# iancze/PSOAP

Hardware: AMD Instinct MI355X
Metric: GP lnprob evals/sec (SB2, N=6000) (higher is better)
Workload: dtype f64; 1 GPU; SB2 chunk 20 epochs x 300 px (N=6000), 32 walkers per step per GPU, one chunk per GPU (BASELINE.json configs[2]; configs[3] at 8 GPUs); timed step = H2D of next proposals || eval, D2H of 32 lnprobs, gather; N=6000, components=2, walkers=32, chunks_per_gpu=1, mode=dag, stream_groups=2, parallelism=chunk-sharded x1, RCCL all_gather of walker lnprobs

## Files before the change

include/psoap_gp.h:

```cpp
#ifndef PSOAP_GP_H
#define PSOAP_GP_H

#include <stdint.h>

#ifdef __cplusplus
extern "C" {
#endif

typedef struct psoap_chunk psoap_chunk;

int psoap_version(void);
const char *psoap_last_error(void);
int psoap_device_count(int *count);

enum {
    PSOAP_SHARE_PROCS = 0,
    PSOAP_SHARE_DAG_LAUNCHES = 1,
    PSOAP_SHARE_TAINTED = 2,
    PSOAP_SHARE_RETRIES = 3,
    PSOAP_SHARE_STAGED_FALLBACKS = 4,
    PSOAP_SHARE_STAGED_POLICY = 5,
    PSOAP_SHARE_MOVED_TASKS = 6,
    PSOAP_SHARE_MOVED_XCD = 7,
    PSOAP_SHARE_LOCK_ACQUISITIONS = 8,
// ... 176 lines not shown
int psoap_stream_plan(int P, int lanes, int workers, int scheme, void *out, long long max_tasks, long long *n_tasks,
                      long long *n_slots, long long *n_ctrs, int *scheme_out);
int psoap_stream_tasklog(psoap_chunk *h, int cap, unsigned long long *out, long long max_words);
int psoap_stream_tasks(psoap_chunk *h, void *out, long long max_tasks, long long *n_tasks);

int psoap_chunk_dag_tasks(psoap_chunk *h, void *out, long long max_tasks, long long *n_tasks);

int psoap_dag_plan(int B, int P, int workers, void *out, long long max_tasks, long long *n_tasks,
                   long long *n_slots, long long *n_ctrs, unsigned int *queue_first );
int psoap_dag_plan_sky(int B, int P, const int *first, int workers, void *out, long long max_tasks, long long *n_tasks,
                       long long *n_slots, long long *n_ctrs, unsigned int *queue_first );
int psoap_sky_first(int c, int N, int B, const double *lwl, const double *gp, int *first_out, int *perm_out);
int psoap_sky_order(int c, int N, int B, const double *lwl, const double *gp, int *first_out, int *perm_out, int *cand_out);
int psoap_sky_clip(int c, int N, int B, const double *lwl, const double *gp, int *first_b_out, long long *units_out,
                   int *cand_out);
int psoap_chunk_sky_stats(psoap_chunk *h, long long *out, int n);
int psoap_dag_plan_multi(int B, const int *Ps, int workers, void *out, long long max_tasks,
                         long long *n_tasks, long long *n_slots, long long *n_ctrs,
                         unsigned int *queue_first);
int psoap_dag_plan_aug(int P, int Mt, int Ms, int workers, int scheme, void *tasks_out,
                       long long max_tasks, long long *n_tasks, long long *n_slots,
                       long long *n_ctrs, unsigned int *queue_first);

int psoap_dag_plan_pool(int B, const int *Ps, int workers, int Mt, int Ms, int scheme, void *tasks_out,
                        long long max_tasks, long long *n_tasks, unsigned int *order_out, unsigned int *dep_out,
                        unsigned int *n_main_out, unsigned int *queue_first, int *has_pool, long long *n_ctrs);
int psoap_dag_pick_workers(int B, const int *Ps, int Mt, int compute_units, int max_workers, int *workers);

#ifdef __cplusplus
}
// ... 3 lines not shown
```

psoap_amd/_lib.py:

```python
from __future__ import annotations

import ctypes
import os

import numpy as np

from .build import LIB_PATH

_dp = ctypes.POINTER(ctypes.c_double)
_ip = ctypes.POINTER(ctypes.c_int)
_i32p = ctypes.POINTER(ctypes.c_int32)
_vp = ctypes.c_void_p

K_CLASSES = 7
K_NAMES = ("fill", "panel_update", "potrf", "trsm", "misc", "dag", "grad_contract")


class Timings(ctypes.Structure):
    _fields_ = [("ms", ctypes.c_double * K_CLASSES),
                ("launches", ctypes.c_int64 * K_CLASSES),
                ("flops", ctypes.c_double * K_CLASSES),
                ("bytes", ctypes.c_double * K_CLASSES),
                ("total_ms", ctypes.c_double)]

# ... 105 lines not shown
    "psoap_chunk_get_timings": (ctypes.c_int, [_vp, ctypes.POINTER(Timings)]),
    "psoap_chunk_set_stream_groups": (ctypes.c_int, [_vp, ctypes.c_int]),
    "psoap_chunk_set_mode": (ctypes.c_int, [_vp, ctypes.c_int]),
    "psoap_chunk_dag_tasklog": (ctypes.c_int, [_vp, ctypes.POINTER(ctypes.c_uint64), ctypes.c_longlong]),
    "psoap_chunk_dag_tasks": (ctypes.c_int, [_vp, _vp, ctypes.c_longlong, ctypes.POINTER(ctypes.c_longlong)]),
    "psoap_dag_plan": (ctypes.c_int, [ctypes.c_int, ctypes.c_int, ctypes.c_int, _vp, ctypes.c_longlong,
                                      ctypes.POINTER(ctypes.c_longlong), ctypes.POINTER(ctypes.c_longlong),
                                      ctypes.POINTER(ctypes.c_longlong), ctypes.POINTER(ctypes.c_uint32)]),
    "psoap_dag_plan_sky": (ctypes.c_int, [ctypes.c_int, ctypes.c_int, _ip, ctypes.c_int, _vp, ctypes.c_longlong,
                                          ctypes.POINTER(ctypes.c_longlong), ctypes.POINTER(ctypes.c_longlong),
                                          ctypes.POINTER(ctypes.c_longlong), ctypes.POINTER(ctypes.c_uint32)]),
    "psoap_sky_first": (ctypes.c_int, [ctypes.c_int, ctypes.c_int, ctypes.c_int, _dp, _dp, _ip, _ip]),
    "psoap_sky_order": (ctypes.c_int, [ctypes.c_int, ctypes.c_int, ctypes.c_int, _dp, _dp, _ip, _ip, _ip]),
    "psoap_sky_clip": (ctypes.c_int, [ctypes.c_int, ctypes.c_int, ctypes.c_int, _dp, _dp, _ip, ctypes.POINTER(ctypes.c_longlong),
                                      _ip]),
    "psoap_chunk_sky_stats": (ctypes.c_int, [_vp, ctypes.POINTER(ctypes.c_longlong), ctypes.c_int]),
    "psoap_dag_plan_multi": (ctypes.c_int, [ctypes.c_int, _ip, ctypes.c_int, _vp, ctypes.c_longlong,
                                      ctypes.POINTER(ctypes.c_longlong), ctypes.POINTER(ctypes.c_longlong),
                                      ctypes.POINTER(ctypes.c_longlong), ctypes.POINTER(ctypes.c_uint32)]),
    "psoap_dag_plan_aug": (ctypes.c_int, [ctypes.c_int, ctypes.c_int, ctypes.c_int, ctypes.c_int, ctypes.c_int, _vp,
                                          ctypes.c_longlong, ctypes.POINTER(ctypes.c_longlong),
                                          ctypes.POINTER(ctypes.c_longlong), ctypes.POINTER(ctypes.c_longlong),
                                          ctypes.POINTER(ctypes.c_uint32)]),
    "psoap_dag_pick_workers": (ctypes.c_int, [ctypes.c_int, _ip, ctypes.c_int, ctypes.c_int, ctypes.c_int, _ip]),
    "psoap_dag_plan_pool": (ctypes.c_int, [ctypes.c_int, _ip, ctypes.c_int, ctypes.c_int, ctypes.c_int, ctypes.c_int, _vp,
                                           ctypes.c_longlong, ctypes.POINTER(ctypes.c_longlong), ctypes.POINTER(ctypes.c_uint32),
                                           ctypes.POINTER(ctypes.c_uint32), ctypes.POINTER(ctypes.c_uint32),
                                           ctypes.POINTER(ctypes.c_uint32), _ip, ctypes.POINTER(ctypes.c_longlong)]),
}

# ... 106 lines not shown
```

psoap_amd/chunk.py:

```python
from __future__ import annotations

import ctypes

import numpy as np

from . import _lib
from ._lib import K_NAMES, Timings, as_f64, check, dptr


class LooResult:
    __slots__ = ("lnp", "loo_logp", "pix_mean", "pix_var", "pix_logp", "pix_z", "ep_resid", "ep_chi2", "ep_logp", "ep_npix")

    def __init__(self, lnp, loo_logp, pix_mean, pix_var, pix_logp, fl, ep_resid=None, ep_chi2=None, ep_logp=None, ep_npix=None):
        self.lnp, self.loo_logp = lnp, loo_logp
        self.pix_mean, self.pix_var, self.pix_logp = pix_mean, pix_var, pix_logp
        with np.errstate(invalid="ignore"):
            self.pix_z = (np.asarray(fl, dtype=np.float64) - pix_mean) / np.sqrt(pix_var)
        self.ep_resid, self.ep_chi2, self.ep_logp, self.ep_npix = ep_resid, ep_chi2, ep_logp, ep_npix

    @classmethod
    def degenerate(cls, N, ep_npix=None):
        nan = lambda n: np.full(n, np.nan)
        if ep_npix is None:
            return cls(-np.inf, np.nan, nan(N), nan(N), nan(N), nan(N))
# ... 403 lines not shown
    def predict_timings(self) -> dict:
        t = _lib.PredictTimings()
        check(self._L.psoap_chunk_predict_timings(self._h, ctypes.byref(t)), "psoap_chunk_predict_timings")
        return t.as_dict()

    def timings(self) -> dict:
        t = Timings()
        check(self._L.psoap_chunk_get_timings(self._h, ctypes.byref(t)), "psoap_chunk_get_timings")
        out = {"total_ms": t.total_ms}
        for k, name in enumerate(K_NAMES):
            out[name] = {"ms": t.ms[k], "launches": int(t.launches[k]), "flops": t.flops[k], "bytes": t.bytes[k]}
        return out

    def sky_stats(self) -> dict:
        names = ("tiles_planned", "tiles_dense", "units_planned", "units_dense", "plan_builds", "cache_hits", "skyline_on",
                 "units_clipped")
        out = (ctypes.c_longlong * len(names))()
        n = self._L.psoap_chunk_sky_stats(self._h, out, len(names))
        if n != len(names):
            raise _lib.PsoapError(f"psoap_chunk_sky_stats reports {n} fields, psoap_amd.chunk names {len(names)}")
        return dict(zip(names, (int(v) for v in out)))


class StreamPipeline:

    def __init__(self, handle: ChunkHandle, c: int, walkers: int, groups: int = 2, scheme: int = -1, submit=None):
        if walkers % groups:
            raise ValueError("walkers must be a multiple of groups")
        self.h, self.c, self.walkers, self.groups = handle, int(c), int(walkers), int(groups)
        self.rows = [slice(g * walkers // groups, (g + 1) * walkers // groups) for g in range(groups)]
        handle.stream_open(c, walkers, scheme)
# ... 115 lines not shown
```

psoap_amd/csrc/dag_kernel.hpp:

```cpp
#pragma once
#include "dag_task.hpp"

#include "chol_kernels.hpp"
#include "fill_kernels.hpp"
#include "potrf_blocked.hpp"
#include "potrf_spine.hpp"
#include "orbit_kernels.hpp"

namespace psoap {

struct alignas(64) MatFlags {
    int rows_done;
    int potrf_done;
    int cnt[2];
    int next_done;
    int off1_ready;
    int step_w[4];
    int cnt3;
    int pad[5];
    int xcol[256][2];
    int rvrow[256];
};
static_assert(sizeof(MatFlags) == 64 + 2048 + 1024, "one cache line of row state + the per-column progress words");

// ... 152 lines not shown
    int* cnt = M3 ? (q % 3 == 2 ? &f->cnt3 : &f->cnt[q % 3]) : &f->cnt[q & 1];
    const int old = __hip_atomic_fetch_add(cnt, n, PSOAP_RLX_AGENT);
    if (old + n == ntasks_row) {
        __builtin_amdgcn_fence(__ATOMIC_ACQ_REL, "agent");
        asm volatile("s_waitcnt vmcnt(0)" ::: "memory");
        __hip_atomic_store(cnt, 0, PSOAP_RLX_AGENT);
        asm volatile("s_waitcnt vmcnt(0)" ::: "memory");
        if (ctl && q > 0) dag_spin_ge(&f->rows_done, q, ctl, 11u);
        __hip_atomic_store(&f->rows_done, q + 1, __ATOMIC_RELEASE, __HIP_MEMORY_SCOPE_AGENT);
    }
}

template <bool SW = false, class SM = SmemKernel, bool ROWMAP = false, bool TD = false>
__device__ __forceinline__ void dag_update(Tile& t, double* Km, int ld, int k0, int j0, int pa, int pb, MatFlags* f,
                                           DagCtl* ctl, bool wait_next, unsigned long long* tl, int wave_s = -1, SM sm = SM(),
                                           int* wa = nullptr, int* wb = nullptr, int ka = 0)
{
    if (pb <= pa) return;
    ka = ka > pa ? ka : pa;
    const bool diag = (k0 == j0);
    unsigned long long w0 = 0;
    if (tl && threadIdx.x == 0) w0 = __builtin_amdgcn_s_memrealtime();
    if (pb - pa > 1) {
        if constexpr (TD) dag_wait_ge2(wa, wb, pb - 1, ctl, 1u);
        else dag_wait_ge(&f->rows_done, pb - 1, ctl, 1u);
        if (tl && threadIdx.x == 0) {
            const unsigned long long w1 = __builtin_amdgcn_s_memrealtime();
            tl[7] += (w1 - w0) << 40;
        }
        const size_t r0 = (size_t)ka * NB;
        tile_gemm_tn<SW, SM, ROWMAP>(t, Km + r0 * ld + k0, (size_t)ld, Km + r0 * ld + j0, (size_t)ld, (pb - 1 - ka) * NB, diag, 0x7fffffff, wave_s, sm);
    }
    if (tl && threadIdx.x == 0) w0 = __builtin_amdgcn_s_memrealtime();
    if constexpr (TD) dag_wait_ge2(wa, wb, pb, ctl, 2u);
    else dag_wait_ge(wait_next ? &f->next_done : &f->rows_done, pb, ctl, 2u);
    if (tl && threadIdx.x == 0) {
        const unsigned long long w1 = __builtin_amdgcn_s_memrealtime();
        tl[4] = w1;
        tl[7] += (w1 - w0) << 40;
    }
    const size_t r1 = (size_t)(pb - 1) * NB;
    if (ka < pb) tile_gemm_tn<SW, SM, ROWMAP>(t, Km + r1 * ld + k0, (size_t)ld, Km + r1 * ld + j0, (size_t)ld, NB, diag, 0x7fffffff, wave_s, sm);
}

template <class SM>
__device__ __forceinline__ void dag_update_following(Tile& t, const double* __restrict__ A, const double* __restrict__ B,
                                                     size_t ld, int* xa, int* xb, int base, unsigned int* err, int wave, SM sm,
                                                     unsigned long long* tl = nullptr)
{
    const int wr = wave >> 1, wc = wave & 1;
    const int lane = hw_lane();
    int avail = ps::x_wait(xa, xb, base, err, 1, lane);
    if (tl && threadIdx.x == 0) tl[4] = __builtin_amdgcn_s_memrealtime();
    __builtin_amdgcn_fence(__ATOMIC_ACQUIRE, "agent");
    stage_glds_w(A, ld, B, ld, 0, 0, wave, sm);
    __syncthreads();
#pragma unroll 1
// ... 1388 lines not shown
#else
        if (LAT && preload && ttype == DAG_DIAG && (task.type & DAG_WAITNEXT) && task.pb - task.pa == 1) {
            dag_diag_fast(Km, ld, k0, Wm, Rv, mat.acc, prev, Npad, f, ctl, q, ntasks_row, (task.type & DAG_FUSED) != 0,
                          &arrive_l[task.ctr], n_wait, dag_opaque_lds(psoap_smem), dag_opaque_lds(vec1), dag_opaque_lds(vec2),
                          tlog_l ? tlog_l + ticket * 8 : nullptr);
            dag_task_end<STREAM>(st, b, mat.acc, mat.P, where0, ctl, wave_s);
            continue;
        }
#endif
        t.zero();
        if (preload) {
            dag_wait_ge(&arrive_l[tctr], n_wait, ctl, 4u);
            dag_sub_partials<false, true>(t, prev, 1);
            n_prev = 0;
        }
        const int ka = __builtin_amdgcn_readfirstlane(ka_v);
        dag_update<true, SmemKernel, false, !LAT && DAG_TILE_DEPS>(
            t, Km, ld, k0, j0, task.pa, task.pb, f, ctl, ttype == DAG_DIAG && (task.type & DAG_WAITNEXT) != 0,
            tlog_l ? tlog_l + ticket * 8 : nullptr, wave_s, SmemKernel(), &f->rvrow[q], &f->rvrow[j], ka);
        if (tlog_l && threadIdx.x == 0) tlog_l[ticket * 8 + 5] = __builtin_amdgcn_s_memrealtime();
        if (!preload && n_wait > 0) dag_wait_ge(&arrive_l[tctr], n_wait, ctl, 4u);
        if (tlog_l && threadIdx.x == 0) tlog_l[ticket * 8 + 6] = __builtin_amdgcn_s_memrealtime();
        dag_sub_partials<false, true>(t, prev, n_prev);
        {
            GpDev g;
            load_gp(mat.gp, C, g);
            double dsum = g.a2[0];
            {
#pragma clang fp contract(off)
                for (int c = 1; c < C; ++c) dsum = dsum + g.a2[c];
            }
            double* dest = is_part ? (wspace_l + (size_t)task.slot * SLOT) : (Km + (size_t)k0 * ld + j0);
            size_t ldd = is_part ? (size_t)NB : (size_t)ld;
            double* mirror = nullptr;
// ... 82 lines not shown
```

psoap_amd/csrc/plan_abi.hpp:

```cpp
#pragma once
#include <string.h>

#include <algorithm>
#include <vector>

#include "abi_error.hpp"
#include "dag_plan.hpp"
#include "sky_rules.hpp"

using namespace psoap;

static void plan_export(const DagPlan& plan, void* out, long long max_tasks, long long* n_tasks, long long* n_slots,
                        long long* n_ctrs, unsigned int* queue_first)
{
    *n_tasks = (long long)plan.tasks.size();
    if (n_slots) *n_slots = plan.n_slots;
    if (n_ctrs) *n_ctrs = plan.n_ctrs;
    if (queue_first) memcpy(queue_first, plan.queues.first, sizeof plan.queues.first);
    if (out) {
        const long long n = max_tasks < *n_tasks ? max_tasks : *n_tasks;
        memcpy(out, plan.tasks.data(), sizeof(DagTask) * n);
    }
}

// ... 101 lines not shown
    if (c < 1 || c > 3 || N < 1 || B < 1 || !lwl || !gp) FAIL("psoap_sky_clip: bad arguments");
    const int P = round_up(N, NB) / NB;
    int cand = 0;
    sky_host_order(c, N, B, lwl, gp, sky_n_cand(c), nullptr, nullptr, &cand);
    std::vector<int> perm, first, first_b;
    if (N <= SKY_MAX_N) sky_host_candidate(c, N, B, lwl, gp, cand, perm, first, &first_b);
    else first_b.assign((size_t)B * P, 0);
    long long units = 0;
    for (int b = 0; b < B; ++b) units += sky_cost(first_b.data() + (size_t)b * P, P);
    if (first_b_out) memcpy(first_b_out, first_b.data(), sizeof(int) * (size_t)B * P);
    if (units_out) *units_out = units;
    if (cand_out) *cand_out = cand;
    return 0;
}

extern "C" int psoap_stream_plan(int P, int lanes, int workers, int scheme, void* out, long long max_tasks,
                                 long long* n_tasks, long long* n_slots, long long* n_ctrs, int* scheme_out)
{
    if (P < 1 || P > 255 || lanes < 1 || lanes > STREAM_MAX_LANES || workers < 1 || scheme < -1 || scheme > 2 || !n_tasks)
        FAIL("psoap_stream_plan: bad arguments");
    if (scheme < 0) scheme = dag_auto_scheme(std::vector<int>((size_t)lanes, P));
    DagPlan plan = dag_build_lane_plan(P, lanes, workers, scheme);
    plan_export(plan, out, max_tasks, n_tasks, n_slots, n_ctrs, nullptr);
    if (scheme_out) *scheme_out = plan.scheme;
    return 0;
}

extern "C" int psoap_dag_plan_aug(int P, int Mt, int Ms, int workers, int scheme, void* out, long long max_tasks,
                                  long long* n_tasks, long long* n_slots, long long* n_ctrs, unsigned int* queue_first)
{
// ... 45 lines not shown
```

psoap_amd/csrc/psoap_gp.hip:

```cpp
#include "../../include/psoap_gp.h"

#include <math.h>
#include <stdio.h>
#include <stdlib.h>
#include <stddef.h>
#include <string.h>

#include <errno.h>
#include <time.h>
#include <unistd.h>

#include <algorithm>
#include <atomic>
#include <chrono>
#include <memory>
#include <mutex>
#include <set>
#include <string>
#include <vector>

#include "chol_kernels.hpp"
#include "dag_kernel.hpp"
#include "solo_kernel.hpp"
#include "dag_launch.hpp"
// ... 39 lines not shown
    return hipDeviceGetPCIBusId(bus, (int)sizeof bus, device) == hipSuccess ? std::string(bus) : std::string();
}

struct BatchSlot {
    Grow<double> dLwl;
    Grow<double> dGp;
    Grow<double> dLwlS;
    Grow<double> dFlS;
    Grow<double> dSigmaS;
    Grow<int> dPerm;
    Grow<int> dCand;
    Grow<int> dFirstB;
    Grow<int, true> hFirst;
    Grow<int> dFirstW;
    Grow<long long, true> hClipUnits;
    Grow<int> dTooFast;
    bool toofast_dirty = false;
    Grow<DagMat> dMats;
    int mats_B = 0, mats_C = 0;
    bool mats_sorted = false;
    bool sky_valid = false;
    int B = 0, C = 0;
    double mu = 1.0;
    std::vector<char> neg;
    Event evUpload;
    Event evEval;
};

namespace psoap { struct PredictWs; struct GradWs; struct FisherWs; struct LooWs; struct MargWs; }

// ... 47 lines not shown
    Grow<double> dVel;
    Grow<double> dOut;
    Grow<double> dDates;
    Grow<double> dPorb;
    Grow<double, true> hPorb;
    Grow<unsigned int, true> hDagErr;
    int mode = 1;
    int dag_grid = 0, n_cus = 0;
    DagWorkspace dag;
    int plan_B = 0, plan_workers = 0;
    bool sky = false;
    bool sky_order = true;
    bool sky_clip = true;
    std::vector<int> plan_first;
    DagPlanWork plan_work;
    long long clip_units = -1;
    struct SkyPlan {
        int B;
        std::vector<int> first;
        DagPlan plan;
        int workers;
        DagPlanWork work;
        Grow<DagTask> dTasks;
    };
    std::vector<SkyPlan> sky_cache;
    long long sky_stats[8] = {};
    Grow<unsigned long long> dTlog;
    long long tlog_tasks = 0;
    Grow<double, true> hLwl, hGp, hVel, hOut;
    BatchSlot slot[2];
    int act = -1;
    int pend = -1;
    Stream own_copy;
    hipStream_t copy() const { return own_copy.s ? own_copy.s : streams[0].s; }
    Event evStaging;
    Event evLast;
    bool last_recorded = false;
    int groups = 2;
    Stream streams[MAX_GROUPS];
    Event evDone[MAX_GROUPS];
    bool profiling = false;
// ... 130 lines not shown
    NEED(h->dR, nb * h->Npad);
    NEED(h->dAcc, ACC_ROWS * nb);
    NEED(h->dOut, nb);
    NEED(h->dPorb, nb * 13);
    NEED(h->hPorb, nb * 13);
    NEED(h->hLwl, nb * 3 * N);
    NEED(h->hGp, nb * 6);
    NEED(h->hOut, nb);
    {
        const char* e = getenv("PSOAP_SKYLINE");
        h->sky = N <= SKY_MAX_N && !(e && e[0] == '0');
        e = getenv("PSOAP_SKY_ORDER");
        h->sky_order = !(e && e[0] == '0');
        e = getenv("PSOAP_SKY_CLIP");
        h->sky_clip = !(e && e[0] == '0');
    }
    const size_t n_cand = h->sky_order ? SKY_MAX_CAND : 1;
    for (BatchSlot& sl : h->slot) {
        if (h->sky) {
            NEED(sl.dLwlS, nb * 3 * N);
            NEED(sl.dFlS, N);
            NEED(sl.dSigmaS, N);
            NEED(sl.dPerm, n_cand * N);
            NEED(sl.dCand, 1);
            HIP_TRY(hipMemset(sl.dCand, 0, sizeof(int)));
            NEED(sl.dFirstB, n_cand * nb * h->P);
            NEED(sl.hFirst, h->P);
            memset(sl.hFirst, 0, sizeof(int) * h->P);
            NEED(sl.dFirstW, nb * h->P);
            HIP_TRY(hipMemset(sl.dFirstW, 0, sizeof(int) * nb * h->P));
            NEED(sl.hClipUnits, 1);
            sl.hClipUnits[0] = 0;
        }
        NEED(sl.dLwl, nb * 3 * N);
        NEED(sl.dGp, nb * 6);
        NEED(sl.dTooFast, nb);
        HIP_TRY(hipMemset(sl.dTooFast, 0, sizeof(int) * nb));
        NEED(sl.dMats, nb);
        HIP_TRY(sl.evUpload.create());
        HIP_TRY(sl.evEval.create());
    }
    const size_t tiles = nb * (size_t)h->P * (h->P + 1) / 2;
    HIP_TRY(h->dag.ctl.need(sizeof(DagCtl) + sizeof(MatFlags) * nb + sizeof(int) * (tiles + 16 + (9 * tiles + 1024) / 32 + 8)));
    NEED(h->hDagErr, 16);
    h->hDagErr[0] = 0;
    if (int rc = dag_workers(h->device, &h->dag_grid, &h->n_cus)) return rc;
    HIP_TRY(h->streams[0].create());
// ... 107 lines not shown
        HIP_TRY(hipMemset(h->dTlog, 0, sizeof(unsigned long long) * 8 * tasks));
        h->tlog_tasks = tasks;
        return 0;
    }
    if (out) {
        const long long n = max_tasks < tasks ? max_tasks : tasks;
        HIP_TRY(hipMemcpy(out, h->dTlog, sizeof(unsigned long long) * 8 * n, hipMemcpyDeviceToHost));
    }
    return 0;
}


extern "C" int psoap_chunk_sky_stats(psoap_chunk* h, long long* out, int n)
{
    if (!h || !out || n < 0) FAIL("psoap_chunk_sky_stats: bad arguments");
    for (int i = 0; i < n && i < 8; ++i) out[i] = h->sky_stats[i];
    return 8;
}

extern "C" int psoap_chunk_dag_tasks(psoap_chunk* h, void* out, long long max_tasks, long long* n_tasks)
{
    if (!h || !n_tasks) FAIL("bad arguments");
    DEVICE_SCOPE(h->device);
    if (set_dev(h)) return 1;
    *n_tasks = h->dag.n_tasks;
    if (out && h->dag.tasks) {
        const long long n = max_tasks < (long long)h->dag.n_tasks ? max_tasks : (long long)h->dag.n_tasks;
        HIP_TRY(hipMemcpy(out, h->dag.tasks, sizeof(DagTask) * n, hipMemcpyDeviceToHost));
    }
    return 0;
}

// ... 54 lines not shown
{
    return h->mode == 1 && h->P <= 255 && !dag_fixed_plan() && dag_lnlike_scheme(std::vector<int>((size_t)B, h->P)) == 0;
}

static int upload_end(psoap_chunk* h, BatchSlot& sl)
{
    HIP_TRY(hipMemcpyAsync(sl.dGp, h->hGp, sizeof(double) * (size_t)sl.B * 2 * sl.C, hipMemcpyHostToDevice, h->copy()));
    sl.sky_valid = h->sky && sky_batch(h, sl.B);
    if (sl.sky_valid) {
        const int N = h->N, rows = sl.B * sl.C;
        hipStream_t s = h->copy();
        const int K = h->sky_order ? sky_n_cand(sl.C) : 1;
        hipLaunchKernelGGL(k_sky_perm, dim3((N + 255) / 256, K), dim3(256), 0, s, sl.dLwl, sl.C, N, sl.dPerm);
        hipLaunchKernelGGL(k_sky_first, dim3(sl.B, K), dim3(256), 0, s, sl.dLwl, sl.dPerm, sl.dGp, sl.C, N, h->P, sl.dFirstB);
        hipLaunchKernelGGL(k_sky_choose, dim3(1), dim3(256), 0, s, sl.dFirstB, sl.B, h->P, K, sl.hFirst, sl.dCand,
                           sl.dFirstW, sl.hClipUnits);
        hipLaunchKernelGGL(k_sky_gather, dim3((N + 255) / 256, rows + 2), dim3(256), 0, s, sl.dPerm, sl.dCand, N, rows, sl.dLwl,
                           sl.dLwlS, h->dFl, sl.dFlS, h->dSigma, sl.dSigmaS);
        HIP_TRY(hipGetLastError());
    }
    HIP_TRY(hipEventRecord(h->evStaging, h->copy()));
    HIP_TRY(hipEventRecord(sl.evUpload, h->copy()));
    return 0;
}

extern "C" int psoap_batch_upload(psoap_chunk* h, int B, int c, const double* lwl, const double* gp, double mu_GP)
{
    if (!h || !lwl || !gp) FAIL("psoap_batch_upload: bad arguments");
    DEVICE_SCOPE(h->device);
    if (set_dev(h)) return 1;
    BatchSlot* sl = nullptr;
// ... 184 lines not shown
    m.lw = lw + (size_t)b * C * h->N;
    m.gp = gp + (size_t)b * 2 * C;
    m.sigma = sigma;
    m.acc = h->dAcc + (size_t)b * ACC_ROWS;
    m.N = h->N;
    m.Npad = h->Npad;
    m.P = h->P;
    m.ld = h->ld;
    return m;
}

static void fill_mats(const psoap_chunk* h, const BatchSlot& sl, DagMat* out, bool sorted)
{
    for (int b = 0; b < sl.B; ++b) {
        out[b] = chunk_mat(h, b, sl.C, sorted ? sl.dLwlS : sl.dLwl, sl.dGp, sorted ? sl.dSigmaS : h->dSigma);
        if (sorted && h->sky_clip) out[b].first = sl.dFirstW + (size_t)b * h->P;
    }
}

static int promote_slot(psoap_chunk* h, const char* who)
{
    if (h->pend >= 0) {
        h->act = h->pend;
        h->pend = -1;
    }
    if (h->act < 0 || h->slot[h->act].B < 1) {
        g_err = std::string(who) + ": nothing uploaded";
        return 2;
    }
    return 0;
}
// ... 19 lines not shown
    const std::vector<int> Ps((size_t)B, P);
    std::vector<int> first;
    const bool sky_on = h->sky && sl.sky_valid && sky_batch(h, B);
    if (sky_on) {
        HIP_TRY(hipEventSynchronize(sl.evUpload));
        bool any = false;
        for (int j = 0; j < P; ++j) {
            const int f = sl.hFirst[j];
            if (f < 0 || f > (j > 0 ? j - 1 : 0) || (j > 0 && f < sl.hFirst[j - 1])) FAIL("psoap_batch_eval: the slot's skyline is not a monotone envelope");
            any = any || f > 0;
        }
        if (any) first.assign(sl.hFirst.p, sl.hFirst.p + P);
    }
    if (int rc = ensure_slot_mats(h, sl, !first.empty())) return rc;
    h->clip_units = !first.empty() && h->sky_clip ? sl.hClipUnits[0] : -1;
    long long units_dense = 0;
    for (int q = 0; q < P; ++q) units_dense += (long long)q * (P - q);
    h->sky_stats[1] = (long long)B * P * (P + 1) / 2;
    h->sky_stats[3] = (long long)B * units_dense;
    h->sky_stats[6] = sky_on ? 1 : 0;
    auto report = [h] {
        const bool dense = h->plan_first.empty();
        h->sky_stats[0] = dense ? h->sky_stats[1] : h->plan_work.tiles;
        h->sky_stats[2] = dense ? h->sky_stats[3] : h->plan_work.units;
        h->sky_stats[7] = h->clip_units >= 0 ? h->clip_units : h->sky_stats[2];
    };
    if (h->plan_B == B && h->plan_first == first) {
        if (!first.empty()) h->sky_stats[5] += 1;
        report();
        return 0;
    }
    h->plan_B = 0;
    if (first.empty()) {
        HIP_TRY(hipStreamSynchronize(h->streams[0]));
        const DagPlan plan = dag_lnlike_plan(Ps, h->n_cus, h->dag_grid, &h->plan_workers);
        h->sky_stats[4] += 1;
        HIP_TRY(h->dag.load(plan, (size_t)h->max_batch));
    } else {
        size_t at = 0;
        while (at < h->sky_cache.size() && !(h->sky_cache[at].B == B && h->sky_cache[at].first == first)) ++at;
// ... 82 lines not shown
        HIP_TRY(hipGetLastError());
        HIP_TRY(hipMemsetAsync(h->dag.ctl, 0, h->dag.ctl_bytes, s));
        static const int poison = getenv("PSOAP_DEBUG_POISON") ? atoi(getenv("PSOAP_DEBUG_POISON")) : 0;
        if (poison & 1) HIP_TRY(hipMemsetAsync(h->dK, 0xFF, sizeof(double) * h->mat_stride * (size_t)B, s));
        if (poison & 2)
            for (int b = 0; b < B; ++b)
                HIP_TRY(hipMemsetAsync(h->dWt + (size_t)b * WT_STRIDE + (size_t)2 * NB * NB, 0xFF, sizeof(double) * MB_DOUBLES, s));
        if ((poison & 4) && h->dag.n_slots) HIP_TRY(hipMemsetAsync(h->dag.ws, 0xFF, sizeof(double) * NB * NB * (size_t)h->dag.n_slots, s));
        if (poison & 8) HIP_TRY(hipMemsetAsync(h->dAcc, 0xFF, sizeof(MatAcc) * ACC_ROWS * (size_t)B, s));
        return 0;
        })) return rc;
    double fl = 0.0;
    for (int q = 0; q < P; ++q) fl += 2.0 * NB * NB * ((double)q * NB * (P - q) + (double)NB * (P - q - 1));
    if (int rc = prof_launch(h, s, PSOAP_K_DAG,
                             h->plan_first.empty() ? fl * B
                                                     : h->plan_work.flops - 2.0 * NB * NB * NB * (double)(h->clip_units >= 0 ? h->plan_work.units - h->clip_units : 0),
                             0.0,
                             [&] { launch_lnlike(h, h->dag, h->plan_workers, C, sl.dMats, B, P, s, h->dTlog); }))
        return rc;
    if (int rc = dag_tail(h, s, h->dag.dag_ctl(), true)) return rc;
    g_share.dag_launches += 1;
    return 0;
}

static int eval_staged(psoap_chunk* h);

extern "C" int psoap_batch_eval(psoap_chunk* h)
{
    if (!h) FAIL("psoap_batch_eval: null handle");
    DEVICE_SCOPE(h->device);
    if (set_dev(h)) return 1;
// ... 2292 lines not shown
```

psoap_amd/csrc/sky_kernels.hpp:

```cpp
#pragma once
#include "common.hpp"
#include "sky_rules.hpp"

namespace psoap {

__global__ __launch_bounds__(256) void k_sky_perm(const double* __restrict__ x, int C, int N, int* __restrict__ perm)
{
    __shared__ unsigned long long keys[1024];
    const int cand = blockIdx.y;
    double w[3];
    sky_cand_weights(C, cand, w);
    auto key = [&](int i) {
        double v[3] = {0.0, 0.0, 0.0};
        for (int c = 0; c < C; ++c) v[c] = x[(size_t)c * N + i];
        return sky_key(sky_cand_key(C, w, v));
    };
    const int i = blockIdx.x * 256 + threadIdx.x;
    const unsigned long long mine = i < N ? key(i) : 0ull;
    int rank = 0;
    for (int k0 = 0; k0 < N; k0 += 1024) {
        __syncthreads();
        for (int k = threadIdx.x; k < 1024; k += 256) keys[k] = k0 + k < N ? key(k0 + k) : ~0ull;
        __syncthreads();
#pragma unroll 16
// ... 50 lines not shown
            hi[idx] = nan ? __builtin_inf() : z;
        }
    }
    __syncthreads();
    double p2[3] = {0.0, 0.0, 0.0};
    const bool ok = sky_gp(gp + (size_t)b * 2 * C, C, p2);
    if ((int)threadIdx.x < P) fb[threadIdx.x] = sky_first_raw((int)threadIdx.x, P, C, lo, hi, p2, ok);
    __syncthreads();
    if (threadIdx.x == 0) sky_first_finish(fb, P);
    __syncthreads();
    if ((int)threadIdx.x < P) first_b[((size_t)cand * B + b) * P + threadIdx.x] = fb[threadIdx.x];
}

__global__ __launch_bounds__(256) void k_sky_choose(const int* __restrict__ first_b, int B, int P, int K,
                                                    int* __restrict__ first_host, int* __restrict__ cand_out,
                                                    int* __restrict__ first_w, long long* __restrict__ units_host)
{
    __shared__ int fu[SKY_MAX_CAND * SKY_MAX_P];
    __shared__ long long cost[SKY_MAX_CAND];
    __shared__ unsigned long long units;
    __shared__ int win;
    if (threadIdx.x == 0) units = 0ull;
    for (int idx = threadIdx.x; idx < K * P; idx += 256) {
        const int k = idx / P, j = idx % P;
        const int* f = first_b + (size_t)k * B * P + j;
        int m = f[0];
        for (int b = 1; b < B; ++b) m = f[(size_t)b * P] < m ? f[(size_t)b * P] : m;
        fu[idx] = m;
    }
    __syncthreads();
    if ((int)threadIdx.x < K) cost[threadIdx.x] = sky_cost(fu + threadIdx.x * P, P);
    __syncthreads();
    if (threadIdx.x == 0) {
        int best = 0;
        for (int k = 1; k < K; ++k) best = cost[k] < cost[best] ? k : best;
        win = best;
        cand_out[0] = best;
    }
    __syncthreads();
    for (int j = threadIdx.x; j < P; j += 256) first_host[j] = fu[win * P + j];
    const int* fw = first_b + (size_t)win * B * P;
    for (int idx = threadIdx.x; idx < B * P; idx += 256) first_w[idx] = fw[idx];
    for (int b = threadIdx.x; b < B; b += 256) atomicAdd(&units, (unsigned long long)sky_cost(fw + (size_t)b * P, P));
    __syncthreads();
    if (threadIdx.x == 0) units_host[0] = (long long)units;
}

}
```

psoap_amd/csrc/sky_rules.hpp:

```cpp
#pragma once
#include "tile_consts.hpp"

namespace psoap {

constexpr int SKY_MAX_N = 8192;
constexpr int SKY_MAX_P = SKY_MAX_N / NB;
constexpr int SKY_MAX_CAND = 15;

PSOAP_HD inline unsigned long long sky_key(double x)
{
    const unsigned long long u = __builtin_bit_cast(unsigned long long, x);
    return (u >> 63) ? ~u : (u | 0x8000000000000000ull);
}

PSOAP_HD inline int sky_n_cand(int C) { return C == 2 ? 9 : C == 3 ? 15 : 1; }

PSOAP_HD inline void sky_cand_weights(int C, int k, double* w)
{
    w[0] = 1.0;
    w[1] = w[2] = 0.0;
    if (C == 2) {
        w[0] = 1.0 - k / 8.0;
        w[1] = k / 8.0;
    } else if (C == 3) {
// ... 77 lines not shown
    if (!ok) return 0;
    int q = 0;
    while (q < j && sky_tile_zero(q, j, P, C, lo, hi, p2)) ++q;
    return q;
}

PSOAP_HD inline void sky_first_finish(int* first, int P)
{
    for (int j = 0; j < P; ++j) {
        const int cap = j > 0 ? j - 1 : 0;
        first[j] = first[j] < cap ? first[j] : cap;
    }
    for (int j = P - 2; j >= 0; --j) first[j] = first[j] < first[j + 1] ? first[j] : first[j + 1];
}

}
```

Measured before the change: 1831 evals/s.

## Refine skyline clipping to KB-row groups inside each tile column

```diff
diff --git a/include/psoap_gp.h b/include/psoap_gp.h
--- a/include/psoap_gp.h
+++ b/include/psoap_gp.h
@@ -214,6 +214,8 @@
 int psoap_sky_order(int c, int N, int B, const double *lwl, const double *gp, int *first_out, int *perm_out, int *cand_out);
 int psoap_sky_clip(int c, int N, int B, const double *lwl, const double *gp, int *first_b_out, long long *units_out,
                    int *cand_out);
+int psoap_sky_clip16(int c, int N, int B, const double *lwl, const double *gp, int *first16_b_out, long long *stages_out,
+                     int *cand_out);
 int psoap_chunk_sky_stats(psoap_chunk *h, long long *out, int n);
 int psoap_dag_plan_multi(int B, const int *Ps, int workers, void *out, long long max_tasks,
                          long long *n_tasks, long long *n_slots, long long *n_ctrs,
diff --git a/psoap_amd/_lib.py b/psoap_amd/_lib.py
--- a/psoap_amd/_lib.py
+++ b/psoap_amd/_lib.py
@@ -143,6 +143,8 @@
     "psoap_sky_order": (ctypes.c_int, [ctypes.c_int, ctypes.c_int, ctypes.c_int, _dp, _dp, _ip, _ip, _ip]),
     "psoap_sky_clip": (ctypes.c_int, [ctypes.c_int, ctypes.c_int, ctypes.c_int, _dp, _dp, _ip, ctypes.POINTER(ctypes.c_longlong),
                                       _ip]),
+    "psoap_sky_clip16": (ctypes.c_int, [ctypes.c_int, ctypes.c_int, ctypes.c_int, _dp, _dp, _ip, ctypes.POINTER(ctypes.c_longlong),
+                                        _ip]),
     "psoap_chunk_sky_stats": (ctypes.c_int, [_vp, ctypes.POINTER(ctypes.c_longlong), ctypes.c_int]),
     "psoap_dag_plan_multi": (ctypes.c_int, [ctypes.c_int, _ip, ctypes.c_int, _vp, ctypes.c_longlong,
                                       ctypes.POINTER(ctypes.c_longlong), ctypes.POINTER(ctypes.c_longlong),
diff --git a/psoap_amd/chunk.py b/psoap_amd/chunk.py
--- a/psoap_amd/chunk.py
+++ b/psoap_amd/chunk.py
@@ -441,7 +441,7 @@
 
     def sky_stats(self) -> dict:
         names = ("tiles_planned", "tiles_dense", "units_planned", "units_dense", "plan_builds", "cache_hits", "skyline_on",
-                 "units_clipped")
+                 "units_clipped", "stages_clipped")
         out = (ctypes.c_longlong * len(names))()
         n = self._L.psoap_chunk_sky_stats(self._h, out, len(names))
         if n != len(names):
diff --git a/psoap_amd/csrc/dag_kernel.hpp b/psoap_amd/csrc/dag_kernel.hpp
--- a/psoap_amd/csrc/dag_kernel.hpp
+++ b/psoap_amd/csrc/dag_kernel.hpp
@@ -190,10 +190,10 @@
 template <bool SW = false, class SM = SmemKernel, bool ROWMAP = false, bool TD = false>
 __device__ __forceinline__ void dag_update(Tile& t, double* Km, int ld, int k0, int j0, int pa, int pb, MatFlags* f,
                                            DagCtl* ctl, bool wait_next, unsigned long long* tl, int wave_s = -1, SM sm = SM(),
-                                           int* wa = nullptr, int* wb = nullptr, int ka = 0)
+                                           int* wa = nullptr, int* wb = nullptr, int ka16 = 0)
 {
     if (pb <= pa) return;
-    ka = ka > pa ? ka : pa;
+    const int r0 = pa * NB > ka16 * KB ? pa * NB : ka16 * KB;
     const bool diag = (k0 == j0);
     unsigned long long w0 = 0;
     if (tl && threadIdx.x == 0) w0 = __builtin_amdgcn_s_memrealtime();
@@ -204,8 +204,7 @@
             const unsigned long long w1 = __builtin_amdgcn_s_memrealtime();
             tl[7] += (w1 - w0) << 40;
         }
-        const size_t r0 = (size_t)ka * NB;
-        tile_gemm_tn<SW, SM, ROWMAP>(t, Km + r0 * ld + k0, (size_t)ld, Km + r0 * ld + j0, (size_t)ld, (pb - 1 - ka) * NB, diag, 0x7fffffff, wave_s, sm);
+        tile_gemm_tn<SW, SM, ROWMAP>(t, Km + (size_t)r0 * ld + k0, (size_t)ld, Km + (size_t)r0 * ld + j0, (size_t)ld, (pb - 1) * NB - r0, diag, 0x7fffffff, wave_s, sm);
     }
     if (tl && threadIdx.x == 0) w0 = __builtin_amdgcn_s_memrealtime();
     if constexpr (TD) dag_wait_ge2(wa, wb, pb, ctl, 2u);
@@ -216,7 +215,7 @@
         tl[7] += (w1 - w0) << 40;
     }
     const size_t r1 = (size_t)(pb - 1) * NB;
-    if (ka < pb) tile_gemm_tn<SW, SM, ROWMAP>(t, Km + r1 * ld + k0, (size_t)ld, Km + r1 * ld + j0, (size_t)ld, NB, diag, 0x7fffffff, wave_s, sm);
+    if (r0 < pb * NB) tile_gemm_tn<SW, SM, ROWMAP>(t, Km + r1 * ld + k0, (size_t)ld, Km + r1 * ld + j0, (size_t)ld, NB, diag, 0x7fffffff, wave_s, sm);
 }
 
 template <class SM>
@@ -1635,10 +1634,10 @@
             dag_sub_partials<false, true>(t, prev, 1);
             n_prev = 0;
         }
-        const int ka = __builtin_amdgcn_readfirstlane(ka_v);
+        const int ka16 = __builtin_amdgcn_readfirstlane(ka_v);
         dag_update<true, SmemKernel, false, !LAT && DAG_TILE_DEPS>(
             t, Km, ld, k0, j0, task.pa, task.pb, f, ctl, ttype == DAG_DIAG && (task.type & DAG_WAITNEXT) != 0,
-            tlog_l ? tlog_l + ticket * 8 : nullptr, wave_s, SmemKernel(), &f->rvrow[q], &f->rvrow[j], ka);
+            tlog_l ? tlog_l + ticket * 8 : nullptr, wave_s, SmemKernel(), &f->rvrow[q], &f->rvrow[j], ka16);
         if (tlog_l && threadIdx.x == 0) tlog_l[ticket * 8 + 5] = __builtin_amdgcn_s_memrealtime();
         if (!preload && n_wait > 0) dag_wait_ge(&arrive_l[tctr], n_wait, ctl, 4u);
         if (tlog_l && threadIdx.x == 0) tlog_l[ticket * 8 + 6] = __builtin_amdgcn_s_memrealtime();
diff --git a/psoap_amd/csrc/plan_abi.hpp b/psoap_amd/csrc/plan_abi.hpp
--- a/psoap_amd/csrc/plan_abi.hpp
+++ b/psoap_amd/csrc/plan_abi.hpp
@@ -139,6 +139,45 @@
     return 0;
 }
 
+extern "C" int psoap_sky_clip16(int c, int N, int B, const double* lwl, const double* gp, int* first16_b_out, long long* stages_out,
+                                int* cand_out)
+{
+    if (c < 1 || c > 3 || N < 1 || B < 1 || !lwl || !gp) FAIL("psoap_sky_clip16: bad arguments");
+    const int P = round_up(N, NB) / NB, G = round_up(N, SKY_G) / SKY_G;
+    int cand = 0;
+    sky_host_order(c, N, B, lwl, gp, sky_n_cand(c), nullptr, nullptr, &cand);
+    std::vector<int> perm, first((size_t)P, 0), first_b, first16((size_t)B * P, 0);
+    long long stages = 0;
+    if (N <= SKY_MAX_N) {
+        sky_host_candidate(c, N, B, lwl, gp, cand, perm, first, &first_b);
+        std::vector<double> x((size_t)c * N), lo((size_t)c * P), hi((size_t)c * P), lo16((size_t)c * G), hi16((size_t)c * G);
+        for (int b = 0; b < B; ++b) {
+            for (int k = 0; k < c; ++k) {
+                double* xk = x.data() + (size_t)k * N;
+                for (int r = 0; r < N; ++r) xk[r] = lwl[((size_t)b * c + k) * N + perm[r]];
+                for (int t = 0; t < P; ++t)
+                    sky_interval(xk, t * NB, (t + 1) * NB < N ? (t + 1) * NB : N, &lo[(size_t)k * P + t], &hi[(size_t)k * P + t]);
+                for (int g = 0; g < G; ++g)
+                    sky_interval(xk, g * SKY_G, (g + 1) * SKY_G < N ? (g + 1) * SKY_G : N, &lo16[(size_t)k * G + g],
+                                 &hi16[(size_t)k * G + g]);
+            }
+            double p2[3] = {0.0, 0.0, 0.0};
+            const bool ok = sky_gp(gp + (size_t)b * 2 * c, c, p2);
+            int* f16 = first16.data() + (size_t)b * P;
+            for (int j = 0; j < P; ++j) f16[j] = sky_first16_raw(j, G, P, c, lo16.data(), hi16.data(), lo.data(), hi.data(), p2, ok);
+            sky_first16_finish(f16, P);
+            for (int j = 0; j < P; ++j)
+                if (f16[j] < SKY_GPT * first_b[(size_t)b * P + j]) FAIL("psoap_sky_clip16: a column starts above its own first tile");
+        }
+    }
+    for (int b = 0; b < B; ++b)
+        for (int j = 0; j < P; ++j) stages += sky_stages_col(j, first[j], first16[(size_t)b * P + j]);
+    if (first16_b_out) memcpy(first16_b_out, first16.data(), sizeof(int) * (size_t)B * P);
+    if (stages_out) *stages_out = stages;
+    if (cand_out) *cand_out = cand;
+    return 0;
+}
+
 extern "C" int psoap_stream_plan(int P, int lanes, int workers, int scheme, void* out, long long max_tasks,
                                  long long* n_tasks, long long* n_slots, long long* n_ctrs, int* scheme_out)
 {
diff --git a/psoap_amd/csrc/psoap_gp.hip b/psoap_amd/csrc/psoap_gp.hip
--- a/psoap_amd/csrc/psoap_gp.hip
+++ b/psoap_amd/csrc/psoap_gp.hip
@@ -77,6 +77,8 @@
     Grow<int, true> hFirst;
     Grow<int> dFirstW;
     Grow<long long, true> hClipUnits;
+    Grow<int> dFirst16;
+    Grow<long long, true> hStages16;
     Grow<int> dTooFast;
     bool toofast_dirty = false;
     Grow<DagMat> dMats;
@@ -154,7 +156,9 @@
     bool sky_clip = true;
     std::vector<int> plan_first;
     DagPlanWork plan_work;
+    bool sky_fine = true;
     long long clip_units = -1;
+    long long clip_stages = -1;
     struct SkyPlan {
         int B;
         std::vector<int> first;
@@ -164,7 +168,7 @@
         Grow<DagTask> dTasks;
     };
     std::vector<SkyPlan> sky_cache;
-    long long sky_stats[8] = {};
+    long long sky_stats[9] = {};
     Grow<unsigned long long> dTlog;
     long long tlog_tasks = 0;
     Grow<double, true> hLwl, hGp, hVel, hOut;
@@ -325,6 +329,8 @@
         h->sky_order = !(e && e[0] == '0');
         e = getenv("PSOAP_SKY_CLIP");
         h->sky_clip = !(e && e[0] == '0');
+        e = getenv("PSOAP_SKY_FINE");
+        h->sky_fine = !(e && e[0] == '0');
     }
     const size_t n_cand = h->sky_order ? SKY_MAX_CAND : 1;
     for (BatchSlot& sl : h->slot) {
@@ -342,6 +348,10 @@
             HIP_TRY(hipMemset(sl.dFirstW, 0, sizeof(int) * nb * h->P));
             NEED(sl.hClipUnits, 1);
             sl.hClipUnits[0] = 0;
+            NEED(sl.dFirst16, nb * h->P);
+            HIP_TRY(hipMemset(sl.dFirst16, 0, sizeof(int) * nb * h->P));
+            NEED(sl.hStages16, nb);
+            memset(sl.hStages16, 0, sizeof(long long) * nb);
         }
         NEED(sl.dLwl, nb * 3 * N);
         NEED(sl.dGp, nb * 6);
@@ -479,8 +489,8 @@
 extern "C" int psoap_chunk_sky_stats(psoap_chunk* h, long long* out, int n)
 {
     if (!h || !out || n < 0) FAIL("psoap_chunk_sky_stats: bad arguments");
-    for (int i = 0; i < n && i < 8; ++i) out[i] = h->sky_stats[i];
-    return 8;
+    for (int i = 0; i < n && i < 9; ++i) out[i] = h->sky_stats[i];
+    return 9;
 }
 
 extern "C" int psoap_chunk_dag_tasks(psoap_chunk* h, void* out, long long max_tasks, long long* n_tasks)
@@ -565,7 +575,10 @@
         hipLaunchKernelGGL(k_sky_perm, dim3((N + 255) / 256, K), dim3(256), 0, s, sl.dLwl, sl.C, N, sl.dPerm);
         hipLaunchKernelGGL(k_sky_first, dim3(sl.B, K), dim3(256), 0, s, sl.dLwl, sl.dPerm, sl.dGp, sl.C, N, h->P, sl.dFirstB);
         hipLaunchKernelGGL(k_sky_choose, dim3(1), dim3(256), 0, s, sl.dFirstB, sl.B, h->P, K, sl.hFirst, sl.dCand,
-                           sl.dFirstW, sl.hClipUnits);
+                           sl.dFirstW, sl.hClipUnits, sl.dFirst16);
+        if (h->sky_clip && h->sky_fine)
+            hipLaunchKernelGGL(k_sky_fine, dim3(sl.B), dim3(256), 0, s, sl.dLwl, sl.dPerm, sl.dCand, sl.dGp, sl.C, N, h->P,
+                               sl.dFirstW, sl.dFirst16, sl.hStages16);
         hipLaunchKernelGGL(k_sky_gather, dim3((N + 255) / 256, rows + 2), dim3(256), 0, s, sl.dPerm, sl.dCand, N, rows, sl.dLwl,
                            sl.dLwlS, h->dFl, sl.dFlS, h->dSigma, sl.dSigmaS);
         HIP_TRY(hipGetLastError());
@@ -780,7 +793,7 @@
 {
     for (int b = 0; b < sl.B; ++b) {
         out[b] = chunk_mat(h, b, sl.C, sorted ? sl.dLwlS : sl.dLwl, sl.dGp, sorted ? sl.dSigmaS : h->dSigma);
-        if (sorted && h->sky_clip) out[b].first = sl.dFirstW + (size_t)b * h->P;
+        if (sorted && h->sky_clip) out[b].first = sl.dFirst16 + (size_t)b * h->P;
     }
 }
 
@@ -830,6 +843,11 @@
     }
     if (int rc = ensure_slot_mats(h, sl, !first.empty())) return rc;
     h->clip_units = !first.empty() && h->sky_clip ? sl.hClipUnits[0] : -1;
+    h->clip_stages = -1;
+    if (h->clip_units >= 0) {
+        h->clip_stages = h->sky_fine ? 0 : SKY_GPT * h->clip_units;
+        for (int b = 0; b < B && h->sky_fine; ++b) h->clip_stages += sl.hStages16[b];
+    }
     long long units_dense = 0;
     for (int q = 0; q < P; ++q) units_dense += (long long)q * (P - q);
     h->sky_stats[1] = (long long)B * P * (P + 1) / 2;
@@ -840,6 +858,7 @@
         h->sky_stats[0] = dense ? h->sky_stats[1] : h->plan_work.tiles;
         h->sky_stats[2] = dense ? h->sky_stats[3] : h->plan_work.units;
         h->sky_stats[7] = h->clip_units >= 0 ? h->clip_units : h->sky_stats[2];
+        h->sky_stats[8] = h->clip_stages >= 0 ? h->clip_stages : SKY_GPT * h->sky_stats[2];
     };
     if (h->plan_B == B && h->plan_first == first) {
         if (!first.empty()) h->sky_stats[5] += 1;
@@ -952,7 +971,7 @@
     for (int q = 0; q < P; ++q) fl += 2.0 * NB * NB * ((double)q * NB * (P - q) + (double)NB * (P - q - 1));
     if (int rc = prof_launch(h, s, PSOAP_K_DAG,
                              h->plan_first.empty() ? fl * B
-                                                     : h->plan_work.flops - 2.0 * NB * NB * NB * (double)(h->clip_units >= 0 ? h->plan_work.units - h->clip_units : 0),
+                                                     : h->plan_work.flops - 2.0 * NB * NB * KB * (double)(h->clip_stages >= 0 ? SKY_GPT * h->plan_work.units - h->clip_stages : 0),
                              0.0,
                              [&] { launch_lnlike(h, h->dag, h->plan_workers, C, sl.dMats, B, P, s, h->dTlog); }))
         return rc;
diff --git a/psoap_amd/csrc/sky_kernels.hpp b/psoap_amd/csrc/sky_kernels.hpp
--- a/psoap_amd/csrc/sky_kernels.hpp
+++ b/psoap_amd/csrc/sky_kernels.hpp
@@ -88,7 +88,8 @@
 
 __global__ __launch_bounds__(256) void k_sky_choose(const int* __restrict__ first_b, int B, int P, int K,
                                                     int* __restrict__ first_host, int* __restrict__ cand_out,
-                                                    int* __restrict__ first_w, long long* __restrict__ units_host)
+                                                    int* __restrict__ first_w, long long* __restrict__ units_host,
+                                                    int* __restrict__ first16_w)
 {
     __shared__ int fu[SKY_MAX_CAND * SKY_MAX_P];
     __shared__ long long cost[SKY_MAX_CAND];
@@ -114,10 +115,81 @@
     __syncthreads();
     for (int j = threadIdx.x; j < P; j += 256) first_host[j] = fu[win * P + j];
     const int* fw = first_b + (size_t)win * B * P;
-    for (int idx = threadIdx.x; idx < B * P; idx += 256) first_w[idx] = fw[idx];
+    for (int idx = threadIdx.x; idx < B * P; idx += 256) {
+        first_w[idx] = fw[idx];
+        first16_w[idx] = SKY_GPT * fw[idx];
+    }
     for (int b = threadIdx.x; b < B; b += 256) atomicAdd(&units, (unsigned long long)sky_cost(fw + (size_t)b * P, P));
     __syncthreads();
     if (threadIdx.x == 0) units_host[0] = (long long)units;
 }
 
+__global__ __launch_bounds__(256) void k_sky_fine(const double* __restrict__ lwl, const int* __restrict__ perm,
+                                                  const int* __restrict__ cand, const double* __restrict__ gp, int C, int N, int P,
+                                                  const int* __restrict__ first_w, int* __restrict__ first16_w,
+                                                  long long* __restrict__ stages_host)
+{
+    __shared__ double lo16[3 * SKY_MAX_G], hi16[3 * SKY_MAX_G];
+    __shared__ double lo[3 * SKY_MAX_P], hi[3 * SKY_MAX_P];
+    __shared__ int f16[SKY_MAX_P];
+    __shared__ unsigned long long stages;
+    const int b = blockIdx.x, B = gridDim.x, G = (N + SKY_G - 1) / SKY_G;
+    const double* x = lwl + (size_t)b * C * N;
+    const int* pm = perm + (size_t)cand[0] * N;
+    const int lane = threadIdx.x & 63, wave = threadIdx.x >> 6;
+    if (threadIdx.x == 0) stages = 0ull;
+    for (int base = 4 * wave; base < C * G; base += 16) {
+        const int idx = base + (lane >> 4);
+        const int c = idx / G, g = idx % G, i = g * SKY_G + (lane & 15);
+        double a = __builtin_inf(), z = -__builtin_inf();
+        int nan = 0;
+        if (idx < C * G && i < N) {
+            const double v = x[(size_t)c * N + pm[i]];
+            nan = !(v == v) ? 1 : 0;
+            a = v < a ? v : a;
+            z = v > z ? v : z;
+        }
+        for (int off = 8; off > 0; off >>= 1) {
+            const double a2 = __shfl_xor(a, off), z2 = __shfl_xor(z, off);
+            nan |= __shfl_xor(nan, off);
+            a = a2 < a ? a2 : a;
+            z = z2 > z ? z2 : z;
+        }
+        if ((lane & 15) == 0 && idx < C * G) {
+            lo16[idx] = nan ? -__builtin_inf() : a;
+            hi16[idx] = nan ? __builtin_inf() : z;
+        }
+    }
+    __syncthreads();
+    for (int idx = threadIdx.x; idx < C * P; idx += 256) {
+        const int c = idx / P, t = idx % P;
+        const int g1 = (t + 1) * SKY_GPT < G ? (t + 1) * SKY_GPT : G;
+        double a = __builtin_inf(), z = -__builtin_inf();
+        for (int g = t * SKY_GPT; g < g1; ++g) {
+            a = lo16[c * G + g] < a ? lo16[c * G + g] : a;
+            z = hi16[c * G + g] > z ? hi16[c * G + g] : z;
+        }
+        lo[idx] = a;
+        hi[idx] = z;
+    }
+    __syncthreads();
+    double p2[3] = {0.0, 0.0, 0.0};
+    const bool ok = sky_gp(gp + (size_t)b * 2 * C, C, p2);
+    if ((int)threadIdx.x < P)
+        f16[threadIdx.x] = sky_first16_raw((int)threadIdx.x, G, P, C, lo16, hi16, lo, hi, p2, ok,
+                                           SKY_GPT * first_w[(size_t)b * P + threadIdx.x]);
+    __syncthreads();
+    if (threadIdx.x == 0) sky_first16_finish(f16, P);
+    __syncthreads();
+    if ((int)threadIdx.x < P) {
+        const int j = threadIdx.x;
+        int u = first_w[j];
+        for (int k = 1; k < B; ++k) u = first_w[(size_t)k * P + j] < u ? first_w[(size_t)k * P + j] : u;
+        first16_w[(size_t)b * P + j] = f16[j];
+        atomicAdd(&stages, (unsigned long long)sky_stages_col(j, u, f16[j]));
+    }
+    __syncthreads();
+    if (threadIdx.x == 0) stages_host[b] = (long long)stages;
 }
+
+}
diff --git a/psoap_amd/csrc/sky_rules.hpp b/psoap_amd/csrc/sky_rules.hpp
--- a/psoap_amd/csrc/sky_rules.hpp
+++ b/psoap_amd/csrc/sky_rules.hpp
@@ -115,4 +115,49 @@
     for (int j = P - 2; j >= 0; --j) first[j] = first[j] < first[j + 1] ? first[j] : first[j + 1];
 }
 
+constexpr int SKY_G = KB;
+constexpr int SKY_GPT = NB / SKY_G;
+constexpr int SKY_MAX_G = SKY_MAX_N / SKY_G;
+
+PSOAP_HD inline bool sky_group_zero(int g, int j, int G, int P, int C, const double* lo16, const double* hi16, const double* lo,
+                                    const double* hi, const double* p2)
+{
+#pragma clang fp contract(off)
+    for (int c = 0; c < C; ++c) {
+        const double g1 = lo[c * P + j] - hi16[c * G + g], g2 = lo16[c * G + g] - hi[c * P + j];
+        const double d = g1 > g2 ? g1 : g2;
+        if (!(d > 0.0)) return false;
+        const double a = p2[c] * d * d;
+        if (!(a <= -746.0)) return false;
+    }
+    return true;
 }
+
+PSOAP_HD inline int sky_first16_raw(int j, int G, int P, int C, const double* lo16, const double* hi16, const double* lo,
+                                    const double* hi, const double* p2, bool ok, int g0 = 0)
+{
+    if (!ok) return 0;
+    const int cap = j > 0 ? SKY_GPT * (j - 1) : 0;
+    int g = g0 < cap ? g0 : cap;
+    while (g < cap && sky_group_zero(g, j, G, P, C, lo16, hi16, lo, hi, p2)) ++g;
+    return g;
+}
+
+PSOAP_HD inline void sky_first16_finish(int* first16, int P)
+{
+    for (int j = P - 2; j >= 0; --j) first16[j] = first16[j] < first16[j + 1] ? first16[j] : first16[j + 1];
+}
+
+PSOAP_HD inline long long sky_stages_col(int j, int u, int s)
+{
+    long long n = 0;
+    const int r0 = SKY_GPT * u > s ? SKY_GPT * u : s;
+    for (int q = u + 1; q <= j; ++q) {
+        if (s >= SKY_GPT * q) continue;
+        const int before = SKY_GPT * (q - 1) - r0;
+        n += SKY_GPT + (before > 0 ? before : 0);
+    }
+    return n;
+}
+
+}
```

Result: faster. 1869 evals/s (median of 6 runs) (+2.0%).
